# remyschwab/TetRex

Hardware: AMD Instinct MI355X
Metric: k-mer IBF probes/sec (higher is better)
Workload: dtype u64; 1 GPU; S-IBF-1024; bins_per_gpu=1024, bins_total=1024, hash_funs=3, bin_size_rows=1247045, kmer_bits=20, matrix_bytes_per_gpu=159621760, mask_words=16, parallelism=bin-column shards x1, no collective on the probe path, probe_unit=one k-mer against all 1024 bins (answered by 1 shard(s) together)

## Files before the change

include/txq.h:

```cpp
#ifndef TXQ_H
#define TXQ_H

#include <stddef.h>
#include <stdint.h>

#ifdef __cplusplus
extern "C" {
#endif

#define TXQ_VERSION 1


typedef enum {
    TXQ_OK = 0,
    TXQ_ERR_ARG = -1,
    TXQ_ERR_HIP = -2,
    TXQ_ERR_NOMEM = -3,
    TXQ_ERR_STATE = -4,
    TXQ_ERR_OVERFLOW = -5,
    TXQ_ERR_PROGRAM = -6
} txq_status;

typedef struct txq_index txq_index;

// ... 44 lines not shown

int txq_index_supports_dense(const txq_index* ix);

int txq_index_memory(const txq_index* ix, uint64_t* free_bytes, uint64_t* kept_bytes);

int txq_index_set_tag(txq_index* ix, uint64_t tag);
int txq_index_get_tag(const txq_index* ix, uint64_t* tag);

int txq_index_create_ibf(uint64_t bins, uint64_t bin_size, uint64_t hash_funs, int shard_rank, int n_shards,
                         txq_index** out);
int txq_index_download_words(const txq_index* ix, uint64_t* words, size_t n_words);

int txq_probe(txq_index* ix, const uint64_t* kmers, size_t n, uint64_t* masks);
int txq_probe_device(txq_index* ix, const uint64_t* d_kmers, size_t n, uint64_t* d_masks, uint64_t* d_alive,
                     void* stream);

int txq_count_device(txq_index* ix, const uint64_t* d_values, const uint64_t* d_offsets, size_t n_queries,
                     const uint32_t* d_thresholds, uint64_t* d_hits, uint32_t* d_counts, void* stream);
int txq_count(txq_index* ix, const uint64_t* values, const uint64_t* offsets, size_t n_queries,
              const uint32_t* thresholds, uint64_t* hits, uint32_t* counts);

int txq_count_windows_device(txq_index* ix, const uint64_t* d_values, const uint64_t* d_win_begin, const uint32_t* d_win_len,
                             size_t n_windows, const uint32_t* d_thresholds, uint64_t* d_hits, uint32_t* d_counts, void* stream);
int txq_count_windows(txq_index* ix, const uint64_t* values, size_t n_values, const uint64_t* win_begin, const uint32_t* win_len,
                      size_t n_windows, const uint32_t* thresholds, uint64_t* hits, uint32_t* counts);

uint64_t txq_translate_bound(const uint64_t* rec_offsets, size_t n_records, unsigned k);
int txq_translate_device(const uint8_t* d_seq, const uint64_t* d_rec_offsets, size_t n_records, unsigned k, const uint8_t* d_codes,
                         uint64_t* d_values, uint64_t* d_offsets, void* stream);
int txq_translate(const uint8_t* seq, const uint64_t* rec_offsets, size_t n_records, unsigned k, const uint8_t* codes,
// ... 155 lines not shown
```

tetrex_amd/capi.py:

```python
import ctypes as C
import os

import numpy as np

_HERE = os.path.dirname(os.path.abspath(__file__))
LIB_PATH = os.path.join(_HERE, "libtxq.so")

u64p = C.POINTER(C.c_uint64)
u32p = C.POINTER(C.c_uint32)

TXQ_MERGED_BIN = 0xFFFFFFFFFFFFFFFF

SYMBOLS = [
    "txq_init", "txq_shutdown", "txq_last_error", "txq_device_count",
    "txq_index_upload", "txq_index_upload_subtrees", "txq_index_get_info", "txq_index_free", "txq_index_supports_dense", "txq_index_memory", "txq_index_set_tag", "txq_index_get_tag", "txq_index_create_ibf",
    "txq_index_download_words", "txq_probe", "txq_probe_device", "txq_emplace_device", "txq_count", "txq_count_device",
    "txq_count_windows", "txq_count_windows_device",
    "txq_translate_bound", "txq_translate_device", "txq_translate",
    "txq_translate_windows_bound", "txq_translate_windows_device", "txq_translate_windows", "txq_translate_frames_bound", "txq_translate_frames_device", "txq_translate_frames",
    "txq_frame_window_letters", "txq_frame_window_letters_device",
    "txq_hit_list_device", "txq_edit_search", "txq_edit_search_device",
    "txq_edit_search_long", "txq_edit_search_long_device", "txq_edit_align", "txq_edit_align_device",
    "txq_edit_targets", "txq_edit_targets_device", "txq_edit_targets_long", "txq_edit_targets_long_device",
    "txq_edit_windows", "txq_edit_windows_device", "txq_edit_align_windows", "txq_edit_align_windows_device",
    "txq_edit_window_targets", "txq_edit_window_targets_device",
    "txq_regex_filter", "txq_regex_filter_device",
    "txq_sketch_device", "txq_union_estimates_device", "txq_pair_unions_device", "txq_tree_insert_device",
    "txq_run_programs", "txq_run_programs_device", "txq_session_begin", "txq_session_set_aux_index", "txq_session_stage", "txq_session_end",
    "txq_malloc", "txq_free", "txq_memcpy_h2d", "txq_memcpy_d2h", "txq_synchronize", "txq_host_alloc", "txq_host_free",
]

# ... 35 lines not shown
    if _LIB is None:
        if not os.path.exists(LIB_PATH):
            raise ImportError("%s is missing: build it with `make` (or __graft_entry__.build()); "
                              "tetrex_amd has no CPU fallback" % LIB_PATH)
        L = C.CDLL(LIB_PATH)
        L.txq_last_error.restype = C.c_char_p
        L.txq_init.argtypes = [C.c_int, C.POINTER(C.c_int)]
        L.txq_index_upload.argtypes = [C.POINTER(IndexDesc), C.c_int, C.c_int, C.POINTER(C.c_void_p)]
        L.txq_index_upload_subtrees.argtypes = [C.POINTER(IndexDesc), C.c_int, C.c_int, C.POINTER(C.c_void_p)]
        L.txq_index_get_info.argtypes = [C.c_void_p, C.POINTER(IndexInfo)]
        L.txq_index_free.argtypes = [C.c_void_p]
        L.txq_index_create_ibf.argtypes = [C.c_uint64, C.c_uint64, C.c_uint64, C.c_int, C.c_int, C.POINTER(C.c_void_p)]
        L.txq_index_download_words.argtypes = [C.c_void_p, u64p, C.c_size_t]
        L.txq_probe.argtypes = [C.c_void_p, u64p, C.c_size_t, u64p]
        L.txq_probe_device.argtypes = [C.c_void_p, C.c_void_p, C.c_size_t, C.c_void_p, C.c_void_p, C.c_void_p]
        L.txq_emplace_device.argtypes = [C.c_void_p, C.c_void_p, C.c_void_p, C.c_size_t, C.c_void_p]
        L.txq_count.argtypes = [C.c_void_p, u64p, u64p, C.c_size_t, u32p, u64p, u32p]
        L.txq_count_device.argtypes = [C.c_void_p, C.c_void_p, C.c_void_p, C.c_size_t, C.c_void_p, C.c_void_p, C.c_void_p, C.c_void_p]
        L.txq_count_windows.argtypes = [C.c_void_p, u64p, C.c_size_t, u64p, u32p, C.c_size_t, u32p, u64p, u32p]
        L.txq_count_windows_device.argtypes = [C.c_void_p, C.c_void_p, C.c_void_p, C.c_void_p, C.c_size_t, C.c_void_p, C.c_void_p, C.c_void_p, C.c_void_p]
        L.txq_translate_bound.restype = C.c_uint64
        L.txq_translate_bound.argtypes = [u64p, C.c_size_t, C.c_uint]
        L.txq_translate_device.argtypes = [C.c_void_p, C.c_void_p, C.c_size_t, C.c_uint, C.c_void_p, C.c_void_p, C.c_void_p, C.c_void_p]
        L.txq_translate.argtypes = [C.c_void_p, u64p, C.c_size_t, C.c_uint, C.c_void_p, u64p, u64p]
        L.txq_translate_windows_bound.restype = C.c_uint64
        L.txq_translate_windows_bound.argtypes = [u64p, C.c_size_t, C.c_uint, C.c_uint32, C.c_uint32]
        L.txq_translate_windows_device.argtypes = [C.c_void_p, C.c_void_p, C.c_size_t, C.c_uint, C.c_void_p, C.c_uint32, C.c_uint32, C.c_void_p, C.c_void_p,
                                                   C.c_void_p, C.c_void_p, C.c_void_p, C.c_void_p]
        L.txq_translate_windows.argtypes = [C.c_void_p, u64p, C.c_size_t, C.c_uint, C.c_void_p, C.c_uint32, C.c_uint32, u64p, u64p, u64p, u64p, u32p]
        L.txq_translate_frames_bound.restype = C.c_uint64
# ... 244 lines not shown
        except Exception:
            pass

    @property
    def shard_words(self):
        return int(self.info.shard_words)

    def probe(self, kmers, out=None):
        k = np.ascontiguousarray(kmers, dtype=np.uint64)
        if out is None:
            out = np.zeros((k.size, self.shard_words), dtype=np.uint64)
        assert out.dtype == np.uint64 and out.flags.c_contiguous and out.size == k.size * self.shard_words
        check(lib().txq_probe(self._h, k.ctypes.data_as(u64p), k.size, out.ctypes.data_as(u64p)))
        return out

    def probe_device(self, d_kmers, n, d_masks, d_alive=None, stream=None):
        check(lib().txq_probe_device(self._h, d_kmers, n, d_masks, d_alive, stream))

    def count(self, values, offsets, thresholds, counts=False):
        v = np.ascontiguousarray(values, dtype=np.uint64)
        o = np.ascontiguousarray(offsets, dtype=np.uint64)
        t = np.ascontiguousarray(thresholds, dtype=np.uint32)
        nq = o.size - 1
        if nq < 0 or t.size != nq:
            raise TxqError(-1, "count: %d offsets and %d thresholds" % (o.size, t.size))
        if nq and int(o.max()) > v.size:
            raise TxqError(-1, "count: offsets run past the %d values" % v.size)
        hits = np.zeros((max(nq, 0), self.shard_words), dtype=np.uint64)
        cnt = np.zeros((max(nq, 0), 64 * self.shard_words), dtype=np.uint32) if counts else None
        check(lib().txq_count(self._h, v.ctypes.data_as(u64p), o.ctypes.data_as(u64p), nq, t.ctypes.data_as(u32p),
# ... 815 lines not shown
```

tetrex_amd/csrc/txq_api.hip:

```cpp
#include "../../include/txq.h"
#include "txq_internal.hpp"
#include "txq_hibf_plan.hpp"

#include <algorithm>
#include <cstdarg>
#include <chrono>
#include <cstdio>
#include <cstring>
#include <map>
#include <mutex>
#include <new>
#include <string>
#include <vector>

namespace txq {

static thread_local std::string g_err;
static std::vector<int> g_devices;

static std::mutex g_spare_mutex;
static std::map<int, std::vector<hipStream_t>> g_spare_streams;
hipStream_t take_spare_stream(int device) {
    std::lock_guard<std::mutex> lk(g_spare_mutex);
    auto it = g_spare_streams.find(device);
// ... 43 lines not shown
    k.hibf_unroll = (int)num("TXQ_HIBF_UNROLL", 1);
    k.hibf_store = (int)num("TXQ_HIBF_STORE_KIND", 0) & 3;
#ifdef TXQ_EXPERIMENTS
    k.hibf_store |= (int)num("TXQ_HIBF_STORE", 0) & 112;
#endif
    k.hibf_waves = std::max(0LL, num("TXQ_HIBF_WAVES", 0));
    k.hibf_stack_lds = std::max(2LL, num("TXQ_HIBF_STACK_LDS", 128));
    k.hibf_layout_direct = num("TXQ_HIBF_LAYOUT_DIRECT", 1) != 0;
    k.probe_blocks_per_cu = (int)std::max(1LL, num("TXQ_PROBE_BLOCKS_PER_CU", 256));
    k.probe_unroll = (int)num("TXQ_PROBE_UNROLL", 2);
    k.probe_nt = flag("TXQ_PROBE_NT");
    k.probe_table = is("TXQ_PROBE_TABLE", '0') ? 0 : is("TXQ_PROBE_TABLE", '1') ? 1 : -1;
    k.probe_table_keep = !is("TXQ_PROBE_TABLE_KEEP", '0');
    k.probe_table_fused = !is("TXQ_PROBE_TABLE_FUSED", '0');
    k.probe_table_tile = !is("TXQ_PROBE_TABLE_TILE", '0');
#ifdef TXQ_EXPERIMENTS
    k.probe_experiment = (int)num("TXQ_PROBE_EXPERIMENT", 0) & 3;
#endif
    std::lock_guard<std::mutex> lock(g_knobs_mutex);
    g_knobs = k;
}

int fail(int code, const char* fmt, ...) {
    char buf[512];
    va_list ap;
    va_start(ap, fmt);
    vsnprintf(buf, sizeof buf, fmt, ap);
    va_end(ap);
    g_err = buf;
    return code;
// ... 295 lines not shown
    TXQ_HIP(hipMemcpy2D(words, (size_t)f.shard_words * 8, f.words, (size_t)f.stride * 8, (size_t)f.shard_words * 8,
                        (size_t)f.bin_size, hipMemcpyDeviceToHost));
    return TXQ_OK;
}

int txq_probe_device(txq_index* ix, const uint64_t* d_kmers, size_t n, uint64_t* d_masks, uint64_t* d_alive, void* stream) {
    read_knobs();
    if (!ix) return fail(TXQ_ERR_ARG, "null argument");
    if (int rc = bind_index(ix)) return rc;
    if (!ix || (n && (!d_kmers || !d_masks))) return fail(TXQ_ERR_ARG, "null argument");
    if (n >> 32) return fail(TXQ_ERR_ARG, "at most 2^32-1 k-mers per call");
    hipStream_t s = (hipStream_t)stream;
    if (ix->is_hibf) return hibf_probe(*ix, knobs(), d_kmers, n, d_masks, d_alive, s);
    hipError_t e = probe_flat(*ix, knobs(), d_kmers, n, d_masks, d_alive, s);
    if (e != hipSuccess) return fail_hip(e, "probe kernel launch");
    return TXQ_OK;
}

int txq_probe(txq_index* ix, const uint64_t* kmers, size_t n, uint64_t* masks) {
    if (!ix) return fail(TXQ_ERR_ARG, "null argument");
    if (int rc = bind_index(ix)) return rc;
    if (!ix || (n && (!kmers || !masks))) return fail(TXQ_ERR_ARG, "null argument");
    const size_t W = ix->shard_words;
    if (W == 0 || n == 0) return TXQ_OK;
    size_t chunk = ((size_t)32 << 20) / (W * 8);
    if (chunk > ((size_t)1 << 20)) chunk = (size_t)1 << 20;
    if (chunk < 1024) chunk = 1024;
    if (chunk > n) chunk = n;
    Index::HostPipe& hp = ix->host_pipe;
    for (int i = 0; i < 2; ++i) {
// ... 300 lines not shown
```

tetrex_amd/csrc/txq_internal.hpp:

```cpp
#pragma once
#include "txq_kernels.hpp"
#include "txq_records.hpp"
#include "txq_exec_plan.hpp"
#include "txq_probe_plan.hpp"
#include "txq_buffers.hpp"
#include "../../include/txq.h"
#include <cstdlib>
#include <map>
#include <mutex>
#include <type_traits>
#include <vector>

#define TXQ_HIP(call)                                        \
    do {                                                     \
        hipError_t e_ = (call);                              \
        if (e_ != hipSuccess) return fail_hip(e_, #call);    \
    } while (0)

namespace txq {

template <int... Vs, class F>
inline bool with_value(int v, F&& f) {
    return ((v == Vs ? (f(std::integral_constant<int, Vs>{}), true) : false) || ...);
}
// ... 28 lines not shown
    bool hibf_small = true;
    bool hibf_lane_hash = false;
    bool final_pinned = true;
    bool hibf_layout_fused = true;
    bool hibf_layout_order = true;
    int hibf_steps_per_group = 0, hibf_tile = 0, hibf_unroll = 1, hibf_store = 0;
    long long hibf_waves = 0;
    bool hibf_layout_direct = true;
    long long hibf_stack_lds = 128;
    int probe_blocks_per_cu = 256, probe_unroll = 2;
    bool probe_nt = false;
    int probe_table = -1;
    bool probe_table_keep = true;
    bool probe_table_fused = true;
    bool probe_table_tile = true;
    int probe_experiment = 0;
};
Knobs knobs();
void read_knobs();

struct DeviceMem {
    static int alloc(void** p, size_t bytes) { return (int)hipMalloc(p, bytes); }
    static void free(void* p) { (void)hipFree(p); }
};
struct PinnedMem {
    static int alloc(void** p, size_t bytes) { return (int)hipHostMalloc(p, bytes, hipHostMallocDefault); }
    static void free(void* p) { (void)hipHostFree(p); }
};
struct EventKind { static void destroy(hipEvent_t e) { (void)hipEventDestroy(e); } };
struct StreamKind { static void destroy(hipStream_t s) { (void)hipStreamDestroy(s); } };
// ... 73 lines not shown
    DeviceBuffer<uint32_t> d_counts;
    DeviceBuffer<uint64_t> scratch_dense_kmers;
    DeviceBuffer<uint64_t> scratch_dense_masks;
    DeviceBuffer<uint32_t> scratch_count_acc;
    DeviceBuffer<unsigned char> scratch_count_io;
    DeviceBuffer<uint64_t> kmer_table; uint32_t kmer_table_bits = 0;
    bool kmer_table_refused = false;
    std::mutex table_mutex;
    uint64_t generation = 0;
    struct ProbeTable {
        DeviceBuffer<uint64_t> rows; size_t cap_rows = 0;
        DeviceBuffer<uint32_t> state;
        ProbeKeep keep;
        Event done;
        bool recorded = false, refused = false;
        std::mutex mutex;
    } probe_table;

    struct StagingSet {
        DeviceBuffer<unsigned char> d_blob, d_aux;
        DeviceBuffer<uint64_t> d_masks;
        Event done;
        bool pending = false;
    };
    struct SessionBuffers {
        StagingSet set[2];
        Stream upload;
        Stream side;
        PinnedBuffer<uint64_t> host_final;
        DeviceBuffer<uint64_t> dev_final;
// ... 141 lines not shown
```

tetrex_amd/csrc/txq_probe.hip:

```cpp
#include "txq_internal.hpp"
#include "txq_probe_plan.hpp"
#include <algorithm>
#include <cstdlib>

namespace txq {

typedef uint32_t u32x4 __attribute__((ext_vector_type(4)));

__device__ __forceinline__ u32x4 ld16(const uint64_t* p) { return *reinterpret_cast<const u32x4*>(p); }
__device__ __forceinline__ void st16_stream(uint64_t* p, u32x4 v) {
    __builtin_nontemporal_store(v, reinterpret_cast<u32x4*>(p));
}
__device__ __forceinline__ bool nonzero(u32x4 v) { return (v.x | v.y | v.z | v.w) != 0u; }

__device__ __forceinline__ void store_chunk(const IbfDev& f, uint64_t* masks, size_t kidx, uint32_t c, u32x4 acc) {
    uint64_t* dst = masks + kidx * f.shard_words + 2u * c;
    if (2u * c + 1u < f.shard_words) st16_stream(dst, acc);
    else __builtin_nontemporal_store(((uint64_t)acc.y << 32) | acc.x, dst);
}

struct NoRoot { static constexpr bool kActive = false; };
struct TreeRoot {
    static constexpr bool kActive = true;
    HibfNode root;
    const ChildRec* children;
    uint32_t wpr_log2;
};

struct TableArgs {
    uint64_t* table;
    uint32_t* state;
    uint32_t ratio, cap_rows;
    uint32_t cap;
    uint32_t fresh, sampled;
    ProbeSlots slot;
    uint32_t experiment;
    uint32_t table_tile;
};
__device__ __forceinline__ ProbeRows table_rows(const TableArgs& T) {
    const uint32_t* acc = T.state + T.slot.acc;
    return table_rows(T.fresh != 0, T.state[T.slot.valid_read], acc[0], acc[1], T.ratio, kDomainSample, T.cap_rows);
}
__device__ __forceinline__ ProbeExtend answer_rows(const TableArgs& T) {
    if (T.sampled) {
        const uint32_t rows = table_rows(T).rows;
        return ProbeExtend{rows, rows};
    }
    const uint32_t* stat = T.state + T.slot.stat_read;
    return extend_rows(T.state[T.slot.valid_read], stat[0], stat[1], T.ratio, T.cap_rows);
}
enum ProbeMode { kPlain = 0, kBuild = 1, kAnswer = 2 };

// ... 122 lines not shown
            }
        }
        if (alive) {
            const uint64_t bits = __ballot(my_alive && mine < n);
            if (lane == 0) alive[tile] = bits;
        }
#ifdef TXQ_EXPERIMENTS
        if (MODE == kAnswer && (experiment & 2u)) {
            const uint64_t bits = __ballot(sink & 1u);
            if (lane == 0) masks[base * f.shard_words] = bits;
        }
#endif
    }
}

template <int LPK, bool WHOLE>
__device__ __forceinline__ void table_tile(const IbfDev& f, uint64_t* __restrict__ masks, uint64_t* __restrict__ alive,
                                           const uint64_t* __restrict__ table, uint32_t row, uint32_t experiment, size_t tile) {
    constexpr int KPS = 64 / LPK;
    constexpr int G = LPK < 8 ? LPK : 8;
    constexpr int GROUPS = LPK / G;
    const int lane = threadIdx.x & 63;
    const int sub = lane % LPK, grp = lane / LPK;
    const bool on = WHOLE || (uint32_t)sub < (f.stride >> 1);
    const size_t base = tile << 6;
    const uint64_t gm = LPK == 64 ? ~0ULL : ((1ULL << LPK) - 1ULL);
    const int my_step = lane / KPS, my_grp = lane % KPS;
    (void)experiment;
#ifdef TXQ_EXPERIMENTS
    uint32_t sink = 0;
#endif
    bool my_alive = false;
    u32x4 x[2][G];
    auto load_group = [&](int g, u32x4* dst) {
        uint32_t r[G];
#pragma unroll
        for (int u = 0; u < G; ++u) r[u] = (uint32_t)__shfl((int)row, (g * G + u) * KPS + grp);
        if constexpr (!WHOLE) {
#pragma unroll
            for (int u = 0; u < G; ++u) dst[u] = u32x4{0u, 0u, 0u, 0u};
        }
#ifdef TXQ_EXPERIMENTS
        if (experiment & 1u) {
#pragma unroll
            for (int u = 0; u < G; ++u) dst[u] = u32x4{0x55555555u, 0x33333333u, 0x0f0f0f0fu, 0x00ff00ffu};
            return;
        }
#endif
        if (on) {
#pragma unroll
            for (int u = 0; u < G; ++u) dst[u] = ld16(table + (size_t)r[u] * f.stride + 2u * sub);
        }
    };
    load_group(0, x[0]);
#pragma unroll
    for (int g = 0; g < GROUPS; ++g) {
        if (g + 1 < GROUPS) load_group(g + 1, x[(g + 1) & 1]);
        __builtin_amdgcn_sched_barrier(0);
        const u32x4* cur = x[g & 1];
        if constexpr (!WHOLE && GROUPS == 1) __builtin_amdgcn_s_waitcnt(0x0F70);
#ifdef TXQ_EXPERIMENTS
        if (experiment & 2u) {
#pragma unroll
            for (int u = 0; u < G; ++u) sink ^= cur[u].x ^ cur[u].y ^ cur[u].z ^ cur[u].w;
        } else
#endif
        if constexpr (WHOLE) {
#pragma unroll
            for (int u = 0; u < G; ++u) st16_stream(masks + (base + (g * G + u) * KPS + grp) * f.shard_words + 2u * sub, cur[u]);
        } else if (on) {
#pragma unroll
            for (int u = 0; u < G; ++u) store_chunk(f, masks, base + (g * G + u) * KPS + grp, sub, cur[u]);
        }
        __builtin_amdgcn_sched_barrier(0);
        if (alive) {
#pragma unroll
            for (int u = 0; u < G; ++u) {
                const uint64_t b = __ballot(on && nonzero(cur[u]));
                if (my_step == g * G + u) my_alive = ((b >> (my_grp * LPK)) & gm) != 0;
            }
        }
    }
    if (alive) {
        const uint64_t bits = __ballot(my_alive);
        if (lane == 0) alive[tile] = bits;
    }
#ifdef TXQ_EXPERIMENTS
    if (experiment & 2u) {
        const uint64_t bits = __ballot(sink & 1u);
        if (lane == 0) masks[base * f.shard_words] = bits;
    }
#endif
}

template <int LPK, int H, int U, bool NT, class ROOT = NoRoot, int MODE = kPlain>
__global__ __launch_bounds__(256) void probe_kernel(IbfDev f, const uint64_t* __restrict__ kmers, size_t n,
                                                    uint64_t* __restrict__ masks, uint64_t* __restrict__ alive, ROOT R = ROOT{},
                                                    TableArgs T = TableArgs{}) {
    const size_t wave = (size_t)blockIdx.x * (blockDim.x >> 6) + (threadIdx.x >> 6);
    const size_t n_waves = (size_t)gridDim.x * (blockDim.x >> 6);
    WaveStats st;
    if constexpr (MODE == kPlain) {
        const size_t n_tiles = (n + 63) >> 6;
        for (size_t tile = wave; tile < n_tiles; tile += n_waves)
            probe_tile<LPK, H, U, NT, ROOT, kPlain>(f, kmers, n, masks, alive, R, nullptr, 0, 0, 0, 0, st, 0, tile);
    } else if constexpr (MODE == kBuild) {
        const ProbeRows tr = table_rows(T);
        const size_t n_tiles = ((size_t)tr.rows + 63) >> 6;
        for (size_t tile = (tr.lo >> 6) + wave; tile < n_tiles; tile += n_waves)
            probe_tile<LPK, H, U, NT, ROOT, kBuild>(f, nullptr, tr.rows, T.table, nullptr, R, nullptr, 0, tr.lo, 0, 0, st, 0, tile);
    } else {
        const ProbeExtend ex = answer_rows(T);
        if (blockIdx.x == 0 && threadIdx.x == 0) {
            T.state[T.slot.valid_write] = ex.rows;
            T.state[T.slot.stat_zero] = 0;
            T.state[T.slot.stat_zero + 1] = 0;
            T.state[T.slot.acc_zero] = 0;
            T.state[T.slot.acc_zero + 1] = 0;
        }
        const size_t n_tiles = (n + 63) >> 6;
        constexpr bool kTableTile = !ROOT::kActive && LPK <= 16;
        const bool tile_ok = kTableTile && T.table_tile && ex.valid;
        const bool whole = (f.stride >> 1) == (uint32_t)LPK && !(f.shard_words & 1u);
        for (size_t tile = wave; tile < n_tiles; tile += n_waves) {
            const size_t mine = (tile << 6) + (threadIdx.x & 63);
            const uint64_t v = mine < n ? __builtin_nontemporal_load(kmers + mine) : 0;
            if constexpr (kTableTile) {
                if (tile_ok && (tile << 6) + 64 <= n && __ballot(v < ex.valid) == ~0ULL) {
                    if (whole) table_tile<LPK, true>(f, masks, alive, T.table, (uint32_t)v, T.experiment, tile);
                    else table_tile<LPK, false>(f, masks, alive, T.table, (uint32_t)v, T.experiment, tile);
                    continue;
                }
            }
            probe_tile<LPK, H, U, NT, ROOT, kAnswer>(f, kmers, n, masks, alive, R, T.table, ex.valid, 0, ex.rows, T.cap, st, T.experiment, tile, v);
        }
        if (st.count && (threadIdx.x & 63) == 0) {
            atomicMax(T.state + T.slot.stat_add, st.top);
            atomicAdd(T.state + T.slot.stat_add + 1, st.count);
        }
        const size_t x_tiles = ((size_t)ex.rows + 63) >> 6;
        for (size_t tile = (ex.valid >> 6) + wave; tile < x_tiles; tile += n_waves)
            probe_tile<LPK, H, U, NT, ROOT, kBuild>(f, nullptr, ex.rows, T.table, nullptr, R, nullptr, 0, ex.valid, 0, 0, st, 0, tile);
    }
}

template <int H>
__global__ __launch_bounds__(256) void probe_w1_kernel(IbfDev f, const uint64_t* __restrict__ kmers, size_t n,
                                                       uint64_t* __restrict__ masks, uint64_t* __restrict__ alive) {
    const size_t stride_threads = (size_t)gridDim.x * blockDim.x;
    const size_t n_pad = (n + 63) & ~(size_t)63;
    for (size_t i = (size_t)blockIdx.x * blockDim.x + threadIdx.x; i < n_pad; i += stride_threads) {
        uint64_t acc = 0;
        if (i < n) {
            const uint64_t v = kmers[i];
            uint64_t w[H];
#pragma unroll
            for (int j = 0; j < H; ++j) w[j] = f.words[hash_row(v, kSeeds[j], f.hash_shift, f.bin_size) * f.stride];
            acc = w[0];
// ... 74 lines not shown
    __shared__ uint32_t s_top[4], s_count[4];
    const int wave = threadIdx.x >> 6;
    if ((threadIdx.x & 63) == 0) {
        s_top[wave] = top;
        s_count[wave] = count;
    }
    __syncthreads();
    if (threadIdx.x == 0) {
        const int waves = blockDim.x >> 6;
        for (int w = 1; w < waves; ++w) {
            top = max(top, s_top[w]);
            count += s_count[w];
        }
        if (top) atomicMax(acc, top);
        if (count) atomicAdd(acc + 1, count);
    }
}


static inline unsigned grid_for(size_t work_items, unsigned per_block) {
    size_t blocks = (work_items + per_block - 1) / per_block;
    const size_t per_cu = (size_t)knobs().probe_blocks_per_cu;
    const size_t cap = 256u * (per_cu ? per_cu : 1);
    if (blocks > cap) blocks = cap;
    if (blocks == 0) blocks = 1;
    return (unsigned)blocks;
}

template <int LPK>
static hipError_t launch_lpk(const IbfDev& f, const uint64_t* k, size_t n, uint64_t* m, uint64_t* a, hipStream_t s) {
// ... 37 lines not shown
        if (!with_hash_funs(f.hash_funs, [&](auto h) { probe_w1_kernel<decltype(h)::value><<<grid, 256, 0, s>>>(f, k, n, m, a); }))
            return hipErrorInvalidValue;
        return hipGetLastError();
    }
    const uint32_t chunks = f.stride >> 1;
    if (chunks <= 1) return launch_lpk<1>(f, k, n, m, a, s);
    if (chunks <= 2) return launch_lpk<2>(f, k, n, m, a, s);
    if (chunks <= 4) return launch_lpk<4>(f, k, n, m, a, s);
    if (chunks <= 8) return launch_lpk<8>(f, k, n, m, a, s);
    if (chunks <= 16) return launch_lpk<16>(f, k, n, m, a, s);
    if (chunks <= 32) return launch_lpk<32>(f, k, n, m, a, s);
    return launch_lpk<64>(f, k, n, m, a, s);
}

template <int LPK>
static hipError_t launch_table_lpk(const IbfDev& f, const uint64_t* k, size_t n, uint64_t* m, uint64_t* a, const TableArgs& T, hipStream_t s) {
    const unsigned bgrid = (unsigned)std::min<size_t>(((size_t)T.cap + 255) / 256, kBuildBlocks);
    const unsigned grid = grid_for((n + 63) / 64, 4);
    if (T.sampled) {
        const uint32_t segs = (uint32_t)std::min<size_t>(std::max<size_t>(n / 1024, 1), 512);
        const size_t head = ((n + segs - 1) / segs + kDomainSample - 1) / kDomainSample;
        const uint32_t parts = (uint32_t)std::max<size_t>((head + 256 * kDomainLoads - 1) / (256 * kDomainLoads), 1);
        probe_domain_kernel<<<segs * parts, 256, 0, s>>>(k, n, T.cap, segs, parts, T.state + T.slot.acc);
    }
    if (f.hash_funs < 2 || !with_hash_funs(f.hash_funs, [&](auto h) {
            constexpr int H = decltype(h)::value;
            if constexpr (H >= 2) {
                if (T.sampled) probe_kernel<LPK, H, 2, false, NoRoot, kBuild><<<bgrid, 256, 0, s>>>(f, nullptr, 0, T.table, nullptr, NoRoot{}, T);
                probe_kernel<LPK, H, 2, false, NoRoot, kAnswer><<<T.sampled ? grid : std::max(grid, bgrid), 256, 0, s>>>(f, k, n, m, a, NoRoot{}, T);
            }
        }))
        return hipErrorInvalidValue;
    return hipGetLastError();
}

hipError_t probe_flat(Index& ix, const Knobs& kn, const uint64_t* k, size_t n, uint64_t* m, uint64_t* a, hipStream_t s) {
    const IbfDev& f = ix.ibf[0];
    const size_t cap = n && f.shard_words ? table_capacity(kn.probe_table, kn.kmer_table_mb, f.bin_size, f.stride, f.hash_funs, n) : 0;
    if (!cap) return launch_probe(f, k, n, m, a, s);
    Index::ProbeTable& pt = ix.probe_table;
    std::lock_guard<std::mutex> lock(pt.mutex);
    if (pt.refused) return launch_probe(f, k, n, m, a, s);
    bool reallocated = false;
// ... 6 lines not shown
            pt.refused = true;
            return launch_probe(f, k, n, m, a, s);
        }
        pt.cap_rows = cap;
        reallocated = true;
    }
    if (pt.recorded) {
        hipError_t e = hipStreamWaitEvent(s, pt.done.get(), 0);
        if (e != hipSuccess) return e;
    }
    const ProbeCall call = plan_probe_call(pt.keep, ix.generation, reallocated, kn.probe_table_keep);
    pt.keep.valid = false;
    if (call.zero_state) {
        hipError_t e = hipMemsetAsync(pt.state.get(), 0, kStateWords * sizeof(uint32_t), s);
        if (e != hipSuccess) return e;
    }
    const bool sampled = call.fresh || !kn.probe_table_fused;
    const TableArgs T{pt.rows.get(), pt.state.get(), kn.probe_table == 1 ? 0u : kTableRatio, (uint32_t)pt.cap_rows, (uint32_t)cap, call.fresh ? 1u : 0u,
                      sampled ? 1u : 0u, probe_slots(pt.keep.calls - 1), (uint32_t)kn.probe_experiment, kn.probe_table_tile ? 1u : 0u};
    const uint32_t chunks = f.stride >> 1;
    hipError_t e;
    if (chunks <= 1) e = launch_table_lpk<1>(f, k, n, m, a, T, s);
    else if (chunks <= 2) e = launch_table_lpk<2>(f, k, n, m, a, T, s);
    else if (chunks <= 4) e = launch_table_lpk<4>(f, k, n, m, a, T, s);
    else if (chunks <= 8) e = launch_table_lpk<8>(f, k, n, m, a, T, s);
    else if (chunks <= 16) e = launch_table_lpk<16>(f, k, n, m, a, T, s);
    else if (chunks <= 32) e = launch_table_lpk<32>(f, k, n, m, a, T, s);
    else e = launch_table_lpk<64>(f, k, n, m, a, T, s);
    if (e != hipSuccess) return e;
    e = hipEventRecord(pt.done.get(), s);
    if (e != hipSuccess) return e;
    pt.recorded = true;
    pt.keep.valid = true;
    return hipSuccess;
}

template <int LPK>
static hipError_t launch_tree_lpk(const IbfDev& f, const TreeRoot& root, const uint64_t* k, size_t n, uint64_t* m, uint64_t* a, hipStream_t s) {
    const unsigned grid = grid_for((n + 63) / 64, 4);
    if (!with_hash_funs(f.hash_funs, [&](auto h) { probe_kernel<LPK, decltype(h)::value, 2, false, TreeRoot><<<grid, 256, 0, s>>>(f, k, n, m, a, root); }))
        return hipErrorInvalidValue;
    return hipGetLastError();
}
// ... 22 lines not shown
```

tetrex_amd/csrc/txq_probe_plan.hpp:

```cpp
#pragma once
#include "txq_records.hpp"
#include <algorithm>
#include <cstddef>

namespace txq {

static constexpr uint32_t kTableRatio = 4;
static constexpr uint32_t kDomainSample = 16;
static constexpr uint32_t kTableMinRows = 1 << 14;
static constexpr size_t kBuildBlocks = 2048;

inline size_t table_capacity(int probe_table, long long table_mb, uint64_t bin_size, uint32_t stride, uint32_t hash_funs, size_t n) {
    if (probe_table == 0 || table_mb <= 0 || (bin_size >> 32) || stride < 2 || (stride & 1) || hash_funs < 2) return 0;
    const size_t budget = ((size_t)table_mb << 20) / ((size_t)stride * 8);
    size_t cap = probe_table == 1 ? std::max<size_t>(n, 1 << 16) : n / kTableRatio;
    cap = std::min(cap, budget) & ~(size_t)63;
    if (probe_table != 1 && cap < kTableMinRows) return 0;
    return cap;
}

struct ProbeRows { uint32_t lo, rows; };
TXQ_HOST_DEVICE inline ProbeRows table_rows(bool fresh, uint32_t built, uint32_t top, uint32_t count, uint32_t ratio, uint32_t sample, uint32_t cap_rows) {
    const uint32_t lo = fresh ? 0u : built < cap_rows ? built : cap_rows;
    const bool pays = top != 0 && top <= cap_rows && (uint64_t)count * sample >= (uint64_t)ratio * top;
    return ProbeRows{lo, pays && top > lo ? top : lo};
}

struct ProbeExtend { uint32_t valid, rows; };
TXQ_HOST_DEVICE inline ProbeExtend extend_rows(uint32_t valid, uint32_t top, uint32_t count, uint32_t ratio, uint32_t cap_rows) {
    const uint32_t V = valid < cap_rows ? valid : cap_rows;
    const bool pays = top > V && top <= cap_rows && (uint64_t)count >= (uint64_t)ratio * (uint64_t)(top - V);
    return ProbeExtend{V, pays ? top : V};
}

enum : uint32_t { kStateAcc = 0, kStateValid = 4, kStateStat = 6, kStateWords = 12 };
struct ProbeSlots {
    uint32_t acc, acc_zero;
    uint32_t valid_read, valid_write;
    uint32_t stat_add, stat_read, stat_zero;
};
inline ProbeSlots probe_slots(uint64_t c) {
    const uint32_t p = (uint32_t)(c & 1), t = (uint32_t)(c % 3);
    return ProbeSlots{kStateAcc + 2u * p, kStateAcc + 2u * (p ^ 1u), kStateValid + p, kStateValid + (p ^ 1u),
                      kStateStat + 2u * t, kStateStat + 2u * ((t + 2u) % 3u), kStateStat + 2u * ((t + 1u) % 3u)};
}

struct ProbeKeep {
    uint64_t generation = 0;
    uint64_t calls = 0;
    bool valid = false;
};
struct ProbeCall {
    bool fresh;
    bool zero_state;
    uint32_t parity;
};
inline ProbeCall plan_probe_call(ProbeKeep& k, uint64_t index_generation, bool reallocated, bool keep) {
    ProbeCall c;
    c.zero_state = !k.valid;
// ... 10 lines not shown
```

Baseline: 26.68 billion probes/s.

## Bucket-sort probe k-mers by table row before answering from kept table

Adds a three-kernel counting sort (histogram, scan, scatter) that groups in-range k-mers by table-row bucket, then answers them with a sorted tile path that reads table rows in bucket order and scatters masks to original positions. Tiles are assigned in an XCD-aware interleave so each XCD works on a contiguous range of buckets. The aim is better cache locality for the random table-row gathers. The cost is extra passes over the k-mers, a scratch records buffer, and scattered mask writes. It runs only when the table is already kept and fused, no alive output is requested, LPK is 8 or 16, and n is at least 8M.

```diff
diff --git a/include/txq.h b/include/txq.h
--- a/include/txq.h
+++ b/include/txq.h
@@ -82,6 +82,7 @@
 int txq_probe(txq_index* ix, const uint64_t* kmers, size_t n, uint64_t* masks);
 int txq_probe_device(txq_index* ix, const uint64_t* d_kmers, size_t n, uint64_t* d_masks, uint64_t* d_alive,
                      void* stream);
+int txq_index_probe_sorted(txq_index* ix, uint64_t out[2]);
 
 int txq_count_device(txq_index* ix, const uint64_t* d_values, const uint64_t* d_offsets, size_t n_queries,
                      const uint32_t* d_thresholds, uint64_t* d_hits, uint32_t* d_counts, void* stream);
diff --git a/tetrex_amd/capi.py b/tetrex_amd/capi.py
--- a/tetrex_amd/capi.py
+++ b/tetrex_amd/capi.py
@@ -14,7 +14,7 @@
 SYMBOLS = [
     "txq_init", "txq_shutdown", "txq_last_error", "txq_device_count",
     "txq_index_upload", "txq_index_upload_subtrees", "txq_index_get_info", "txq_index_free", "txq_index_supports_dense", "txq_index_memory", "txq_index_set_tag", "txq_index_get_tag", "txq_index_create_ibf",
-    "txq_index_download_words", "txq_probe", "txq_probe_device", "txq_emplace_device", "txq_count", "txq_count_device",
+    "txq_index_download_words", "txq_probe", "txq_probe_device", "txq_index_probe_sorted", "txq_emplace_device", "txq_count", "txq_count_device",
     "txq_count_windows", "txq_count_windows_device",
     "txq_translate_bound", "txq_translate_device", "txq_translate",
     "txq_translate_windows_bound", "txq_translate_windows_device", "txq_translate_windows", "txq_translate_frames_bound", "txq_translate_frames_device", "txq_translate_frames",
@@ -80,6 +80,7 @@
         L.txq_index_download_words.argtypes = [C.c_void_p, u64p, C.c_size_t]
         L.txq_probe.argtypes = [C.c_void_p, u64p, C.c_size_t, u64p]
         L.txq_probe_device.argtypes = [C.c_void_p, C.c_void_p, C.c_size_t, C.c_void_p, C.c_void_p, C.c_void_p]
+        L.txq_index_probe_sorted.argtypes = [C.c_void_p, u64p]
         L.txq_emplace_device.argtypes = [C.c_void_p, C.c_void_p, C.c_void_p, C.c_size_t, C.c_void_p]
         L.txq_count.argtypes = [C.c_void_p, u64p, u64p, C.c_size_t, u32p, u64p, u32p]
         L.txq_count_device.argtypes = [C.c_void_p, C.c_void_p, C.c_void_p, C.c_size_t, C.c_void_p, C.c_void_p, C.c_void_p, C.c_void_p]
@@ -354,6 +355,11 @@
         check(lib().txq_probe(self._h, k.ctypes.data_as(u64p), k.size, out.ctypes.data_as(u64p)))
         return out
 
+    def probe_sorted(self):
+        out = (C.c_uint64 * 2)()
+        check(lib().txq_index_probe_sorted(self._h, out))
+        return int(out[0]), int(out[1])
+
     def probe_device(self, d_kmers, n, d_masks, d_alive=None, stream=None):
         check(lib().txq_probe_device(self._h, d_kmers, n, d_masks, d_alive, stream))
 
diff --git a/tetrex_amd/csrc/txq_api.hip b/tetrex_amd/csrc/txq_api.hip
--- a/tetrex_amd/csrc/txq_api.hip
+++ b/tetrex_amd/csrc/txq_api.hip
@@ -81,6 +81,9 @@
     k.probe_table_keep = !is("TXQ_PROBE_TABLE_KEEP", '0');
     k.probe_table_fused = !is("TXQ_PROBE_TABLE_FUSED", '0');
     k.probe_table_tile = !is("TXQ_PROBE_TABLE_TILE", '0');
+    k.probe_sort = !is("TXQ_PROBE_SORT", '0');
+    k.probe_sort_min = std::max(1LL, num("TXQ_PROBE_SORT_MIN", kSortMinDefault));
+    k.probe_sort_bucket_kb = std::max(1LL, num("TXQ_PROBE_SORT_BUCKET_KB", kSortBucketKbDefault));
 #ifdef TXQ_EXPERIMENTS
     k.probe_experiment = (int)num("TXQ_PROBE_EXPERIMENT", 0) & 3;
 #endif
@@ -406,6 +409,22 @@
     if (ix->is_hibf) return hibf_probe(*ix, knobs(), d_kmers, n, d_masks, d_alive, s);
     hipError_t e = probe_flat(*ix, knobs(), d_kmers, n, d_masks, d_alive, s);
     if (e != hipSuccess) return fail_hip(e, "probe kernel launch");
+    return TXQ_OK;
+}
+
+int txq_index_probe_sorted(txq_index* ix, uint64_t out[2]) {
+    if (!ix || !out) return fail(TXQ_ERR_ARG, "null argument");
+    if (int rc = bind_index(ix)) return rc;
+    Index::ProbeTable& pt = ix->probe_table;
+    std::lock_guard<std::mutex> lock(pt.mutex);
+    out[0] = pt.sort_planned;
+    out[1] = 0;
+    if (pt.recorded && pt.state) {
+        uint32_t ran = 0;
+        TXQ_HIP(hipEventSynchronize(pt.done.get()));
+        TXQ_HIP(hipMemcpy(&ran, pt.state.get() + kStateSorted, sizeof ran, hipMemcpyDeviceToHost));
+        out[1] = ran;
+    }
     return TXQ_OK;
 }
 
diff --git a/tetrex_amd/csrc/txq_internal.hpp b/tetrex_amd/csrc/txq_internal.hpp
--- a/tetrex_amd/csrc/txq_internal.hpp
+++ b/tetrex_amd/csrc/txq_internal.hpp
@@ -66,6 +66,9 @@
     bool probe_table_keep = true;
     bool probe_table_fused = true;
     bool probe_table_tile = true;
+    bool probe_sort = true;
+    long long probe_sort_min = kSortMinDefault;
+    long long probe_sort_bucket_kb = kSortBucketKbDefault;
     int probe_experiment = 0;
 };
 Knobs knobs();
@@ -169,6 +172,10 @@
         ProbeKeep keep;
         Event done;
         bool recorded = false, refused = false;
+        DeviceBuffer<uint64_t> sort_records;
+        DeviceBuffer<uint32_t> sort_counts;
+        bool sort_refused = false;
+        uint64_t sort_planned = 0;
         std::mutex mutex;
     } probe_table;
 
diff --git a/tetrex_amd/csrc/txq_probe.hip b/tetrex_amd/csrc/txq_probe.hip
--- a/tetrex_amd/csrc/txq_probe.hip
+++ b/tetrex_amd/csrc/txq_probe.hip
@@ -36,6 +36,9 @@
     ProbeSlots slot;
     uint32_t experiment;
     uint32_t table_tile;
+    const uint64_t* records;
+    uint32_t tiles_per_xcd, sort_blocks;
+    uint32_t outside, outside_zero;
 };
 __device__ __forceinline__ ProbeRows table_rows(const TableArgs& T) {
     const uint32_t* acc = T.state + T.slot.acc;
@@ -188,9 +191,10 @@
     }
 }
 
-template <int LPK, bool WHOLE>
+template <int LPK, bool WHOLE, bool SORTED = false, bool RAGGED = false>
 __device__ __forceinline__ void table_tile(const IbfDev& f, uint64_t* __restrict__ masks, uint64_t* __restrict__ alive,
-                                           const uint64_t* __restrict__ table, uint32_t row, uint32_t experiment, size_t tile) {
+                                           const uint64_t* __restrict__ table, uint32_t row, uint32_t experiment, size_t tile,
+                                           uint32_t dst = 0, uint32_t count = 64) {
     constexpr int KPS = 64 / LPK;
     constexpr int G = LPK < 8 ? LPK : 8;
     constexpr int GROUPS = LPK / G;
@@ -206,24 +210,24 @@
 #endif
     bool my_alive = false;
     u32x4 x[2][G];
-    auto load_group = [&](int g, u32x4* dst) {
+    auto load_group = [&](int g, u32x4* out) {
         uint32_t r[G];
 #pragma unroll
         for (int u = 0; u < G; ++u) r[u] = (uint32_t)__shfl((int)row, (g * G + u) * KPS + grp);
         if constexpr (!WHOLE) {
 #pragma unroll
-            for (int u = 0; u < G; ++u) dst[u] = u32x4{0u, 0u, 0u, 0u};
+            for (int u = 0; u < G; ++u) out[u] = u32x4{0u, 0u, 0u, 0u};
         }
 #ifdef TXQ_EXPERIMENTS
         if (experiment & 1u) {
 #pragma unroll
-            for (int u = 0; u < G; ++u) dst[u] = u32x4{0x55555555u, 0x33333333u, 0x0f0f0f0fu, 0x00ff00ffu};
+            for (int u = 0; u < G; ++u) out[u] = u32x4{0x55555555u, 0x33333333u, 0x0f0f0f0fu, 0x00ff00ffu};
             return;
         }
 #endif
         if (on) {
 #pragma unroll
-            for (int u = 0; u < G; ++u) dst[u] = ld16(table + (size_t)r[u] * f.stride + 2u * sub);
+            for (int u = 0; u < G; ++u) out[u] = ld16(table + (size_t)r[u] * f.stride + 2u * sub);
         }
     };
     load_group(0, x[0]);
@@ -239,7 +243,14 @@
             for (int u = 0; u < G; ++u) sink ^= cur[u].x ^ cur[u].y ^ cur[u].z ^ cur[u].w;
         } else
 #endif
-        if constexpr (WHOLE) {
+        if constexpr (SORTED) {
+            uint32_t to[G];
+#pragma unroll
+            for (int u = 0; u < G; ++u) to[u] = (uint32_t)__shfl((int)dst, (g * G + u) * KPS + grp);
+#pragma unroll
+            for (int u = 0; u < G; ++u)
+                if (!RAGGED || (uint32_t)((g * G + u) * KPS + grp) < count) st16_stream(masks + (size_t)to[u] * f.shard_words + 2u * sub, cur[u]);
+        } else if constexpr (WHOLE) {
 #pragma unroll
             for (int u = 0; u < G; ++u) st16_stream(masks + (base + (g * G + u) * KPS + grp) * f.shard_words + 2u * sub, cur[u]);
         } else if (on) {
@@ -247,7 +258,7 @@
             for (int u = 0; u < G; ++u) store_chunk(f, masks, base + (g * G + u) * KPS + grp, sub, cur[u]);
         }
         __builtin_amdgcn_sched_barrier(0);
-        if (alive) {
+        if (!SORTED && alive) {
 #pragma unroll
             for (int u = 0; u < G; ++u) {
                 const uint64_t b = __ballot(on && nonzero(cur[u]));
@@ -255,7 +266,7 @@
             }
         }
     }
-    if (alive) {
+    if (!SORTED && alive) {
         const uint64_t bits = __ballot(my_alive);
         if (lane == 0) alive[tile] = bits;
     }
@@ -265,6 +276,73 @@
         if (lane == 0) masks[base * f.shard_words] = bits;
     }
 #endif
+}
+
+template <int LPK>
+__device__ __forceinline__ void sorted_tiles(const IbfDev& f, size_t n, uint64_t* __restrict__ masks, const TableArgs& T) {
+    const size_t n_tiles = (n + 63) >> 6;
+    const uint32_t lane = threadIdx.x & 63, wave = threadIdx.x >> 6;
+    for (uint32_t b = blockIdx.x; b < T.sort_blocks; b += gridDim.x) {
+        const size_t tile = (size_t)(b % kSortXcds) * T.tiles_per_xcd + (size_t)(b / kSortXcds) * 4u + wave;
+        if (tile >= n_tiles) continue;
+        const size_t mine = (tile << 6) + lane;
+        if ((tile << 6) + 64 <= n) {
+            const uint64_t rec = __builtin_nontemporal_load(T.records + mine);
+            table_tile<LPK, true, true, false>(f, masks, nullptr, T.table, (uint32_t)(rec >> 32), T.experiment, tile, (uint32_t)rec);
+        } else {
+            const uint64_t rec = mine < n ? __builtin_nontemporal_load(T.records + mine) : 0;
+            table_tile<LPK, true, true, true>(f, masks, nullptr, T.table, (uint32_t)(rec >> 32), T.experiment, tile, (uint32_t)rec,
+                                                       (uint32_t)(n - (tile << 6)));
+        }
+    }
+}
+
+template <int LPK, int H, int U, bool NT, class ROOT, bool SORT>
+__device__ __forceinline__ void answer_body(const IbfDev& f, const uint64_t* __restrict__ kmers, size_t n, uint64_t* __restrict__ masks,
+                                            uint64_t* __restrict__ alive, const ROOT& R, const TableArgs& T) {
+    const size_t wave = (size_t)blockIdx.x * (blockDim.x >> 6) + (threadIdx.x >> 6);
+    const size_t n_waves = (size_t)gridDim.x * (blockDim.x >> 6);
+    WaveStats st;
+    const ProbeExtend ex = answer_rows(T);
+    if (blockIdx.x == 0 && threadIdx.x == 0) {
+        T.state[T.slot.valid_write] = ex.rows;
+        T.state[T.slot.stat_zero] = 0;
+        T.state[T.slot.stat_zero + 1] = 0;
+        T.state[T.slot.acc_zero] = 0;
+        T.state[T.slot.acc_zero + 1] = 0;
+        T.state[T.outside_zero] = 0;
+    }
+    const size_t n_tiles = (n + 63) >> 6;
+    constexpr bool kTableTile = !ROOT::kActive && LPK <= 16;
+    const bool tile_ok = kTableTile && T.table_tile && ex.valid;
+    const bool whole = (f.stride >> 1) == (uint32_t)LPK && !(f.shard_words & 1u);
+    bool sorted = false;
+    if constexpr (SORT) {
+        sorted = T.state[T.outside] == 0;
+        if (sorted) {
+            if (blockIdx.x == 0 && threadIdx.x == 0) atomicAdd(T.state + kStateSorted, 1u);
+            sorted_tiles<LPK>(f, n, masks, T);
+        }
+    }
+    for (size_t tile = sorted ? n_tiles : wave; tile < n_tiles; tile += n_waves) {
+        const size_t mine = (tile << 6) + (threadIdx.x & 63);
+        const uint64_t v = mine < n ? __builtin_nontemporal_load(kmers + mine) : 0;
+        if constexpr (kTableTile) {
+            if (tile_ok && (tile << 6) + 64 <= n && __ballot(v < ex.valid) == ~0ULL) {
+                if (whole) table_tile<LPK, true>(f, masks, alive, T.table, (uint32_t)v, T.experiment, tile);
+                else table_tile<LPK, false>(f, masks, alive, T.table, (uint32_t)v, T.experiment, tile);
+                continue;
+            }
+        }
+        probe_tile<LPK, H, U, NT, ROOT, kAnswer>(f, kmers, n, masks, alive, R, T.table, ex.valid, 0, ex.rows, T.cap, st, T.experiment, tile, v);
+    }
+    if (st.count && (threadIdx.x & 63) == 0) {
+        atomicMax(T.state + T.slot.stat_add, st.top);
+        atomicAdd(T.state + T.slot.stat_add + 1, st.count);
+    }
+    const size_t x_tiles = ((size_t)ex.rows + 63) >> 6;
+    for (size_t tile = (ex.valid >> 6) + wave; tile < x_tiles; tile += n_waves)
+        probe_tile<LPK, H, U, NT, ROOT, kBuild>(f, nullptr, ex.rows, T.table, nullptr, R, nullptr, 0, ex.valid, 0, 0, st, 0, tile);
 }
 
 template <int LPK, int H, int U, bool NT, class ROOT = NoRoot, int MODE = kPlain>
@@ -284,38 +362,16 @@
         for (size_t tile = (tr.lo >> 6) + wave; tile < n_tiles; tile += n_waves)
             probe_tile<LPK, H, U, NT, ROOT, kBuild>(f, nullptr, tr.rows, T.table, nullptr, R, nullptr, 0, tr.lo, 0, 0, st, 0, tile);
     } else {
-        const ProbeExtend ex = answer_rows(T);
-        if (blockIdx.x == 0 && threadIdx.x == 0) {
-            T.state[T.slot.valid_write] = ex.rows;
-            T.state[T.slot.stat_zero] = 0;
-            T.state[T.slot.stat_zero + 1] = 0;
-            T.state[T.slot.acc_zero] = 0;
-            T.state[T.slot.acc_zero + 1] = 0;
-        }
-        const size_t n_tiles = (n + 63) >> 6;
-        constexpr bool kTableTile = !ROOT::kActive && LPK <= 16;
-        const bool tile_ok = kTableTile && T.table_tile && ex.valid;
-        const bool whole = (f.stride >> 1) == (uint32_t)LPK && !(f.shard_words & 1u);
-        for (size_t tile = wave; tile < n_tiles; tile += n_waves) {
-            const size_t mine = (tile << 6) + (threadIdx.x & 63);
-            const uint64_t v = mine < n ? __builtin_nontemporal_load(kmers + mine) : 0;
-            if constexpr (kTableTile) {
-                if (tile_ok && (tile << 6) + 64 <= n && __ballot(v < ex.valid) == ~0ULL) {
-                    if (whole) table_tile<LPK, true>(f, masks, alive, T.table, (uint32_t)v, T.experiment, tile);
-                    else table_tile<LPK, false>(f, masks, alive, T.table, (uint32_t)v, T.experiment, tile);
-                    continue;
-                }
-            }
-            probe_tile<LPK, H, U, NT, ROOT, kAnswer>(f, kmers, n, masks, alive, R, T.table, ex.valid, 0, ex.rows, T.cap, st, T.experiment, tile, v);
-        }
-        if (st.count && (threadIdx.x & 63) == 0) {
-            atomicMax(T.state + T.slot.stat_add, st.top);
-            atomicAdd(T.state + T.slot.stat_add + 1, st.count);
-        }
-        const size_t x_tiles = ((size_t)ex.rows + 63) >> 6;
-        for (size_t tile = (ex.valid >> 6) + wave; tile < x_tiles; tile += n_waves)
-            probe_tile<LPK, H, U, NT, ROOT, kBuild>(f, nullptr, ex.rows, T.table, nullptr, R, nullptr, 0, ex.valid, 0, 0, st, 0, tile);
-    }
+        (void)wave, (void)n_waves, (void)st;
+        answer_body<LPK, H, U, NT, ROOT, false>(f, kmers, n, masks, alive, R, T);
+    }
+}
+
+constexpr int sorted_answer_waves(int lpk, int h) { return lpk == 16 && h == 2 ? 2 : (lpk == 8 && h == 5) || (lpk == 16 && h == 4) ? 3 : 4; }
+template <int LPK, int H>
+__global__ __launch_bounds__(256, sorted_answer_waves(LPK, H)) void probe_sorted_answer_kernel(IbfDev f, const uint64_t* __restrict__ kmers, size_t n, uint64_t* __restrict__ masks,
+                                                                  TableArgs T) {
+    answer_body<LPK, H, 2, false, NoRoot, true>(f, kmers, n, masks, nullptr, NoRoot{}, T);
 }
 
 template <int H>
@@ -420,6 +476,107 @@
         }
         if (top) atomicMax(acc, top);
         if (count) atomicAdd(acc + 1, count);
+    }
+}
+
+struct SortArgs {
+    uint32_t* counts;
+    uint64_t* records;
+    uint32_t shift, buckets, chunks;
+};
+__device__ __forceinline__ uint32_t block_scan256(uint32_t x, uint32_t* wsum, uint32_t& total) {
+    const uint32_t lane = threadIdx.x & 63, wave = threadIdx.x >> 6;
+    uint32_t incl = x;
+#pragma unroll
+    for (int o = 1; o < 64; o <<= 1) {
+        const uint32_t up = (uint32_t)__shfl_up((int)incl, o);
+        if ((int)lane >= o) incl += up;
+    }
+    __syncthreads();
+    if (lane == 63) wsum[wave] = incl;
+    __syncthreads();
+    uint32_t before = 0;
+    total = 0;
+    for (uint32_t w = 0; w < 4; ++w) {
+        if (w < wave) before += wsum[w];
+        total += wsum[w];
+    }
+    return before + incl - x;
+}
+static constexpr int kSortPerThread = kSortChunk / 256;
+
+__global__ __launch_bounds__(256) void probe_sort_count_kernel(const uint64_t* __restrict__ kmers, size_t n, SortArgs S, TableArgs T) {
+    __shared__ uint32_t hist[kSortMaxBuckets];
+    const uint32_t valid = answer_rows(T).valid;
+    if (valid == 0) {
+        if (blockIdx.x == 0 && threadIdx.x == 0) atomicOr(T.state + T.outside, 1u);
+        return;
+    }
+    hist[threadIdx.x] = 0;
+    __syncthreads();
+    const size_t base = (size_t)blockIdx.x * kSortChunk + threadIdx.x;
+    uint64_t v[kSortPerThread];
+#pragma unroll
+    for (int j = 0; j < kSortPerThread; ++j) v[j] = base + j * 256 < n ? __builtin_nontemporal_load(kmers + base + j * 256) : 0;
+    bool out = false;
+#pragma unroll
+    for (int j = 0; j < kSortPerThread; ++j) {
+        if (base + j * 256 >= n) continue;
+        if (v[j] < valid) atomicAdd(&hist[(uint32_t)v[j] >> S.shift], 1u);
+        else out = true;
+    }
+    if (__ballot(out) && (threadIdx.x & 63) == 0) atomicOr(T.state + T.outside, 1u);
+    __syncthreads();
+    if (threadIdx.x < S.buckets) S.counts[(size_t)threadIdx.x * S.chunks + blockIdx.x] = hist[threadIdx.x];
+}
+
+__global__ __launch_bounds__(256) void probe_sort_scan_kernel(SortArgs S, TableArgs T) {
+    __shared__ uint32_t wsum[4];
+    if (T.state[T.outside]) return;
+    uint32_t* row = S.counts + (size_t)blockIdx.x * S.chunks;
+    uint32_t carry = 0;
+    for (uint32_t c0 = 0; c0 < S.chunks; c0 += 256) {
+        const uint32_t c = c0 + threadIdx.x;
+        const uint32_t x = c < S.chunks ? row[c] : 0;
+        uint32_t total;
+        const uint32_t ex = block_scan256(x, wsum, total);
+        if (c < S.chunks) row[c] = carry + ex;
+        carry += total;
+    }
+    if (threadIdx.x == 0) S.counts[(size_t)S.buckets * S.chunks + blockIdx.x] = carry;
+}
+
+__global__ __launch_bounds__(256) void probe_sort_scatter_kernel(const uint64_t* __restrict__ kmers, size_t n, SortArgs S, TableArgs T) {
+    __shared__ uint32_t hist[kSortMaxBuckets], delta[kSortMaxBuckets], wsum[4];
+    __shared__ uint64_t stage[kSortChunk];
+    if (T.state[T.outside]) return;
+    const uint32_t valid = answer_rows(T).valid;
+    hist[threadIdx.x] = 0;
+    __syncthreads();
+    const size_t base = (size_t)blockIdx.x * kSortChunk + threadIdx.x;
+    uint64_t v[kSortPerThread];
+    uint32_t rank[kSortPerThread];
+#pragma unroll
+    for (int j = 0; j < kSortPerThread; ++j) v[j] = base + j * 256 < n ? __builtin_nontemporal_load(kmers + base + j * 256) : ~0ULL;
+#pragma unroll
+    for (int j = 0; j < kSortPerThread; ++j) rank[j] = v[j] < valid ? atomicAdd(&hist[(uint32_t)v[j] >> S.shift], 1u) : 0u;
+    __syncthreads();
+    const bool mine = threadIdx.x < S.buckets;
+    uint32_t total;
+    const uint32_t bucket_base = block_scan256(mine ? S.counts[(size_t)S.buckets * S.chunks + threadIdx.x] : 0u, wsum, total);
+    const uint32_t local = block_scan256(hist[threadIdx.x], wsum, total);
+    const uint32_t global = mine ? bucket_base + S.counts[(size_t)threadIdx.x * S.chunks + blockIdx.x] : 0u;
+    __syncthreads();
+    hist[threadIdx.x] = local;
+    delta[threadIdx.x] = global - local;
+    __syncthreads();
+#pragma unroll
+    for (int j = 0; j < kSortPerThread; ++j)
+        if (v[j] < valid) stage[hist[(uint32_t)v[j] >> S.shift] + rank[j]] = (v[j] << 32) | (uint32_t)(base + j * 256);
+    __syncthreads();
+    for (uint32_t p = threadIdx.x; p < total; p += 256) {
+        const uint64_t rec = stage[p];
+        S.records[(size_t)(uint32_t)(delta[(uint32_t)(rec >> 32) >> S.shift] + p)] = rec;
     }
 }
 
@@ -487,9 +644,16 @@
 }
 
 template <int LPK>
-static hipError_t launch_table_lpk(const IbfDev& f, const uint64_t* k, size_t n, uint64_t* m, uint64_t* a, const TableArgs& T, hipStream_t s) {
+static hipError_t launch_table_lpk(const IbfDev& f, const uint64_t* k, size_t n, uint64_t* m, uint64_t* a, const TableArgs& T, const SortArgs& S,
+                                   hipStream_t s) {
     const unsigned bgrid = (unsigned)std::min<size_t>(((size_t)T.cap + 255) / 256, kBuildBlocks);
-    const unsigned grid = grid_for((n + 63) / 64, 4);
+    unsigned grid = grid_for((n + 63) / 64, 4);
+    if (T.records) {
+        probe_sort_count_kernel<<<S.chunks, 256, 0, s>>>(k, n, S, T);
+        probe_sort_scan_kernel<<<S.buckets, 256, 0, s>>>(S, T);
+        probe_sort_scatter_kernel<<<S.chunks, 256, 0, s>>>(k, n, S, T);
+        grid = (std::max(std::min<unsigned>(grid, T.sort_blocks), bgrid) + kSortXcds - 1) / kSortXcds * kSortXcds;
+    }
     if (T.sampled) {
         const uint32_t segs = (uint32_t)std::min<size_t>(std::max<size_t>(n / 1024, 1), 512);
         const size_t head = ((n + segs - 1) / segs + kDomainSample - 1) / kDomainSample;
@@ -500,6 +664,12 @@
             constexpr int H = decltype(h)::value;
             if constexpr (H >= 2) {
                 if (T.sampled) probe_kernel<LPK, H, 2, false, NoRoot, kBuild><<<bgrid, 256, 0, s>>>(f, nullptr, 0, T.table, nullptr, NoRoot{}, T);
+                if constexpr (LPK == 8 || LPK == 16) {
+                    if (T.records) {
+                        probe_sorted_answer_kernel<LPK, H><<<grid, 256, 0, s>>>(f, k, n, m, T);
+                        return;
+                    }
+                }
                 probe_kernel<LPK, H, 2, false, NoRoot, kAnswer><<<T.sampled ? grid : std::max(grid, bgrid), 256, 0, s>>>(f, k, n, m, a, NoRoot{}, T);
             }
         }))
@@ -536,19 +706,37 @@
     if (call.zero_state) {
         hipError_t e = hipMemsetAsync(pt.state.get(), 0, kStateWords * sizeof(uint32_t), s);
         if (e != hipSuccess) return e;
+        pt.sort_planned = 0;
     }
     const bool sampled = call.fresh || !kn.probe_table_fused;
+    const uint32_t chunks = f.stride >> 1;
+    const uint32_t lpk = chunks <= 1 ? 1 : chunks <= 2 ? 2 : chunks <= 4 ? 4 : chunks <= 8 ? 8 : chunks <= 16 ? 16 : chunks <= 32 ? 32 : 64;
+    ProbeSort ps = plan_probe_sort(!sampled && kn.probe_table_tile, a != nullptr, false, lpk, f.stride, f.shard_words, n, pt.cap_rows,
+                                   kn.probe_sort && !pt.sort_refused, kn.probe_sort_min, kn.probe_sort_bucket_kb, kn.kmer_table_mb);
+    if (ps.on) {
+        const auto after_last_call = free_after([&pt] { if (pt.recorded) (void)hipEventSynchronize(pt.done.get()); });
+        if (pt.sort_records.reserve(exactly(n * sizeof(uint64_t)), after_last_call) ||
+            pt.sort_counts.reserve(exactly(((size_t)ps.buckets * ps.chunks + kSortMaxBuckets) * sizeof(uint32_t)), after_last_call)) {
+            (void)hipGetLastError();
+            pt.sort_refused = true;
+            ps = ProbeSort{};
+        }
+    }
+    const uint32_t parity = (uint32_t)((pt.keep.calls - 1) & 1);
     const TableArgs T{pt.rows.get(), pt.state.get(), kn.probe_table == 1 ? 0u : kTableRatio, (uint32_t)pt.cap_rows, (uint32_t)cap, call.fresh ? 1u : 0u,
-                      sampled ? 1u : 0u, probe_slots(pt.keep.calls - 1), (uint32_t)kn.probe_experiment, kn.probe_table_tile ? 1u : 0u};
-    const uint32_t chunks = f.stride >> 1;
+                      sampled ? 1u : 0u, probe_slots(pt.keep.calls - 1), (uint32_t)kn.probe_experiment, kn.probe_table_tile ? 1u : 0u,
+                      ps.on ? pt.sort_records.get() : nullptr, (uint32_t)ps.tiles_per_xcd, (uint32_t)ps.blocks,
+                      kStateOutside + parity, kStateOutside + (parity ^ 1u)};
+    const SortArgs S{pt.sort_counts.get(), pt.sort_records.get(), ps.shift, ps.buckets, ps.chunks};
+    if (ps.on) ++pt.sort_planned;
     hipError_t e;
-    if (chunks <= 1) e = launch_table_lpk<1>(f, k, n, m, a, T, s);
-    else if (chunks <= 2) e = launch_table_lpk<2>(f, k, n, m, a, T, s);
-    else if (chunks <= 4) e = launch_table_lpk<4>(f, k, n, m, a, T, s);
-    else if (chunks <= 8) e = launch_table_lpk<8>(f, k, n, m, a, T, s);
-    else if (chunks <= 16) e = launch_table_lpk<16>(f, k, n, m, a, T, s);
-    else if (chunks <= 32) e = launch_table_lpk<32>(f, k, n, m, a, T, s);
-    else e = launch_table_lpk<64>(f, k, n, m, a, T, s);
+    if (chunks <= 1) e = launch_table_lpk<1>(f, k, n, m, a, T, S, s);
+    else if (chunks <= 2) e = launch_table_lpk<2>(f, k, n, m, a, T, S, s);
+    else if (chunks <= 4) e = launch_table_lpk<4>(f, k, n, m, a, T, S, s);
+    else if (chunks <= 8) e = launch_table_lpk<8>(f, k, n, m, a, T, S, s);
+    else if (chunks <= 16) e = launch_table_lpk<16>(f, k, n, m, a, T, S, s);
+    else if (chunks <= 32) e = launch_table_lpk<32>(f, k, n, m, a, T, S, s);
+    else e = launch_table_lpk<64>(f, k, n, m, a, T, S, s);
     if (e != hipSuccess) return e;
     e = hipEventRecord(pt.done.get(), s);
     if (e != hipSuccess) return e;
diff --git a/tetrex_amd/csrc/txq_probe_plan.hpp b/tetrex_amd/csrc/txq_probe_plan.hpp
--- a/tetrex_amd/csrc/txq_probe_plan.hpp
+++ b/tetrex_amd/csrc/txq_probe_plan.hpp
@@ -33,7 +33,7 @@
     return ProbeExtend{V, pays ? top : V};
 }
 
-enum : uint32_t { kStateAcc = 0, kStateValid = 4, kStateStat = 6, kStateWords = 12 };
+enum : uint32_t { kStateAcc = 0, kStateValid = 4, kStateStat = 6, kStateOutside = 12, kStateSorted = 14, kStateWords = 16 };
 struct ProbeSlots {
     uint32_t acc, acc_zero;
     uint32_t valid_read, valid_write;
@@ -43,6 +43,37 @@
     const uint32_t p = (uint32_t)(c & 1), t = (uint32_t)(c % 3);
     return ProbeSlots{kStateAcc + 2u * p, kStateAcc + 2u * (p ^ 1u), kStateValid + p, kStateValid + (p ^ 1u),
                       kStateStat + 2u * t, kStateStat + 2u * ((t + 2u) % 3u), kStateStat + 2u * ((t + 1u) % 3u)};
+}
+
+static constexpr uint32_t kSortChunk = 4096, kSortMaxBuckets = 256, kSortXcds = 8;
+static constexpr long long kSortMinDefault = 1 << 23;
+static constexpr long long kSortBucketKbDefault = 1024;
+struct ProbeSort {
+    bool on = false;
+    uint32_t shift = 0, buckets = 0, chunks = 0;
+    uint64_t n_tiles = 0, tiles_per_xcd = 0, blocks = 0;
+};
+inline uint64_t sort_tile(const ProbeSort& p, uint64_t block, uint32_t wave) {
+    return (block % kSortXcds) * p.tiles_per_xcd + (block / kSortXcds) * 4u + wave;
+}
+inline ProbeSort plan_probe_sort(bool kept_fused, bool has_alive, bool has_root, uint32_t lpk, uint32_t stride, uint32_t shard_words, uint64_t n,
+                                 size_t cap_rows, bool sort, long long sort_min, long long bucket_kb, long long scratch_mb) {
+    ProbeSort p;
+    const bool whole = stride / 2 == lpk && !(stride & 1) && !(shard_words & 1) && shard_words == stride;
+    if (!sort || !kept_fused || has_alive || has_root || lpk < 8 || lpk > 16 || !whole || n == 0 || (n >> 32) || cap_rows == 0 || (cap_rows >> 32) ||
+        sort_min < 1 || n < (uint64_t)sort_min || scratch_mb < 0 || n * 8 > ((uint64_t)scratch_mb << 20))
+        return p;
+    const uint64_t row_bytes = (uint64_t)stride * 8;
+    const uint64_t bucket_rows = std::max<uint64_t>(((uint64_t)std::max(bucket_kb, 1LL) << 10) / row_bytes, 1);
+    while ((2ull << p.shift) <= bucket_rows) ++p.shift;
+    while ((((uint64_t)cap_rows - 1) >> p.shift) + 1 > kSortMaxBuckets) ++p.shift;
+    p.buckets = (uint32_t)((((uint64_t)cap_rows - 1) >> p.shift) + 1);
+    p.chunks = (uint32_t)((n + kSortChunk - 1) / kSortChunk);
+    p.n_tiles = (n + 63) >> 6;
+    p.tiles_per_xcd = ((p.n_tiles + kSortXcds - 1) / kSortXcds + 3) & ~(uint64_t)3;
+    p.blocks = kSortXcds * (p.tiles_per_xcd / 4);
+    p.on = true;
+    return p;
 }
 
 struct ProbeKeep {
```

After: 30.73 billion probes/s, median of 6. 15.2% higher.
